# re-ovo/wgpu-path-tracing

Hardware: AMD Instinct MI355X
Metric: Msamples/s (rays x bounces / s) (higher is better)
Workload: dtype f32

## Files before the change

### wgpu-path-tracing_amd/csrc/dispatch.hip

```cpp
#include "ptmi_ctx.h"

#include <algorithm>
#include <cmath>
#include <cstring>
#include <utility>
#include <vector>

namespace {

constexpr size_t kMaxPendingEvents = 4096;
constexpr size_t kMaxDispatchesInFlight = 256;

const struct { double ptmi_stats::*ms; uint64_t ptmi_stats::*launches; } kEventStat[kEventKinds] = {
    {&ptmi_stats::gpu_ms, nullptr},
    {&ptmi_stats::extend_ms, &ptmi_stats::extend_launches},
    {&ptmi_stats::shade_ms, &ptmi_stats::shade_launches},
    {&ptmi_stats::shadow_ms, &ptmi_stats::shadow_launches},
    {&ptmi_stats::raygen_ms, nullptr},
    {&ptmi_stats::compact_ms, nullptr},
    {&ptmi_stats::accumulate_ms, nullptr},
};

hipEvent_t get_event(ptmi_ctx *c) {
    if (!c->event_pool.empty()) { hipEvent_t e = c->event_pool.back(); c->event_pool.pop_back(); return e; }
// ... 135 lines not shown
        float4 *const aov_rec = c->aov_mask ? ln.aov : nullptr;
        float4 *const mom = plane_as<float4>(c, kMoments);
        unsigned long long *const ct = c->d_counters;
        uint32_t *const qlen = &c->d_control[kCwQueue], *const slen = &c->d_control[kCwShadow];
        if (ap && !map && cam->frame_index == 0u) { pt_launch_adaptive_restart(ms, blocks, band, mom); c->ad_rounds = 0; }
        auto batch = [&](uint32_t frame0, uint32_t fb) -> int {
            const DevPixels px = ap ? DevPixels{band, 0u, c->ad.list, &c->d_control[kCwAdActive], mom, &ct[kCtAdTraced]}
                                    : DevPixels{band, frame0, nullptr, nullptr, nullptr, nullptr};
            { Timed t(c, kRaygen, t3, ms); pt_launch_raygen(ms, blocks, *cam, px, fb, bp, &qlen[0]); }
            int cur = 0;
            for (uint32_t b = 0; b < maxb; b++) {
                const bool tail = b > rb;
                const uint32_t *q = b == 0 || b == rb + 1 ? nullptr : ln.queue[cur];
                const DevPaths sp = tail ? tp : bp;
                const int par = side ? (int)(b & 1u) : 0;
                const ShadeParams shp{b, maxb, c->opt.do_mis, ct, side ? 1u : 0u, tail ? ln.pid : nullptr};
                { Timed t(c, kExtend, t2, ms); launch_extend(c, ms, cfg, sp, q, &qlen[b], ln.hits);
                  if (alpha) alpha_resolve_paths(c, ms, cfg, sp, q, &qlen[b], ln.hits, nullptr); }
                const bool last = b + 1 == maxb;
                if (side && b >= 2) HIP_TRY(c, hipStreamWaitEvent(ms, ln.ev_shadow[par], 0));
                { Timed t(c, kShade, t3, ms);
                  (c->opt.perf_mode ? pt_launch_shade_fast : pt_launch_shade)(
                      ms, shade_blocks, c->sc, sp, q, &qlen[b], ln.hits, ln.sh[par], ln.alive, ln.shadowm, shp,
                      b == 0 ? aov_rec : nullptr); }
                { Timed t(c, kCompact, t3, ms);
                  pt_launch_compact(ms, tiles, q, &qlen[b], ln.alive, nee ? ln.shadowm : nullptr,
                                    ln.word_off, ln.queue[cur ^ 1], &qlen[b + 1], ln.sq[par], &slen[par],
                                    ct, b, last ? 0 : 1);
                  if (b == rb && !last) pt_launch_repack(ms, blocks, &qlen[b + 1], ln.queue[cur ^ 1], bp, tp, ln.pid); }
                if (side) {
                    HIP_TRY(c, hipEventRecord(ln.ev_ready, ms));
                    HIP_TRY(c, hipStreamWaitEvent(ss, ln.ev_ready, 0));
                    { Timed t(c, kShadow, t3, ss); launch_shadow(c, ss, cfg_shadow, bp, ln.sh[par], ln.sq[par], &slen[par], nullptr); }
                    HIP_TRY(c, hipEventRecord(ln.ev_shadow[par], ss));
                } else if (nee) {
                    Timed t(c, kShadow, t3, ms);
                    if (alpha) alpha_shadow_stage(c, ms, cfg, bp, ln.sh[0], ln.sq[0], &slen[0], ln.hits, nullptr, nullptr);
                    else launch_shadow(c, ms, cfg_shadow, bp, ln.sh[0], ln.sq[0], &slen[0], nullptr);
                }
                cur ^= 1;
            }
// ... 222 lines not shown
```

### wgpu-path-tracing_amd/csrc/pipeline.hip

```cpp
#include "pt_device.h"
#include "pt_math.h"

namespace {

constexpr int BLOCK = 256;

PT_DEV v3 camera_dir(const ptmi_camera &cam, float px, float py) {
    float uvx = (px / (float)cam.width) * 2.0f - 1.0f;
    float uvy = (py / (float)cam.height) * 2.0f - 1.0f;
    float th = tan1(cam.fov * 0.5f);
    v3 fw = mk3(cam.forward[0], cam.forward[1], cam.forward[2]);
    v3 rt = mk3(cam.right[0], cam.right[1], cam.right[2]);
    v3 up = mk3(cam.up[0], cam.up[1], cam.up[2]);
    v3 a = scale3(scale3(scale3(rt, uvx), th), cam.aspect);
    v3 b = scale3(scale3(up, uvy), th);
    return normalize3(add3(add3(fw, a), b));
}

PT_DEV void camera_ray(const ptmi_camera &cam, uint32_t x, uint32_t y, uint32_t frame, v3 &org, v3 &dir,
                       uint32_t &rng) {
    rng = rng_seed(x, y, frame);
    float jx = rng_f(rng), jy = rng_f(rng);
    v3 rt = mk3(cam.right[0], cam.right[1], cam.right[2]);
    v3 up = mk3(cam.up[0], cam.up[1], cam.up[2]);
// ... 63 lines not shown
__global__ __launch_bounds__(BLOCK) void k_raygen_list(ptmi_camera cam, uint32_t n, const uint32_t *xs,
                                                       const uint32_t *ys, const uint32_t *frames, DevPaths P) {
    uint32_t p = blockIdx.x * BLOCK + threadIdx.x;
    if (p >= n) return;
    v3 o, d; uint32_t rng;
    camera_ray(cam, xs[p], ys[p], frames[p], o, d, rng);
    init_path(P, p, o, d, rng);
}

#ifndef PT_TILE_WORDS
#define PT_TILE_WORDS 1024
#endif
constexpr int TILE_WORDS = PT_TILE_WORDS;
constexpr int TILE_WAVES = TILE_WORDS / 64;

__global__ __launch_bounds__(TILE_WORDS) void k_tile_sums(const uint32_t *__restrict__ count_ptr,
                                                          const uint64_t *__restrict__ alive,
                                                          const uint64_t *__restrict__ shadow,
                                                          uint32_t *__restrict__ tile_sums,
                                                          uint32_t *__restrict__ shadow_tile_sums,
                                                          unsigned long long *__restrict__ stats, uint32_t bounce) {
    __shared__ uint32_t wsum[TILE_WAVES], wssum[TILE_WAVES];
    const uint32_t count = *count_ptr;
    const uint32_t nwords = (count + 63u) >> 6;
    if (blockIdx.x == 0 && threadIdx.x == 0) {
        atomicAdd(&stats[kCtSegments], (unsigned long long)count); atomicAdd(&stats[kCtByBounce + bounce], (unsigned long long)count);
    }
    if (blockIdx.x * TILE_WORDS >= nwords) return;
    const uint32_t w = blockIdx.x * TILE_WORDS + threadIdx.x;
    uint32_t c = 0, sc = 0;
    if (w < nwords) { c = (uint32_t)__popcll(alive[w]); if (shadow) sc = (uint32_t)__popcll(shadow[w]); }
    for (int off = 32; off > 0; off >>= 1) { c += __shfl_down(c, off); sc += __shfl_down(sc, off); }
    if ((threadIdx.x & 63u) == 0u) { wsum[threadIdx.x >> 6] = c; wssum[threadIdx.x >> 6] = sc; }
    __syncthreads();
    if (threadIdx.x == 0) {
        uint32_t t = 0, ts = 0;
        for (int i = 0; i < TILE_WAVES; i++) { t += wsum[i]; ts += wssum[i]; }
        tile_sums[blockIdx.x] = t;
        shadow_tile_sums[blockIdx.x] = ts;
        if (ts) { atomicAdd(&stats[kCtShadowRays], (unsigned long long)ts); atomicAdd(&stats[kCtShadowTraced], (unsigned long long)ts); }
    }
}

template <bool PACKED>
PT_DEV void scatter_tile(uint32_t tile, const uint32_t *__restrict__ count_ptr, const uint32_t *__restrict__ queue,
                         const uint64_t *__restrict__ alive, const uint32_t *__restrict__ tile_sums,
                         uint32_t *__restrict__ next_queue, uint32_t *__restrict__ next_count) {
    __shared__ uint32_t wtot[TILE_WAVES];
    __shared__ uint32_t tile_base;
    const uint32_t count = *count_ptr;
    const uint32_t nwords = (count + 63u) >> 6;
    const uint32_t ntiles = (nwords + TILE_WORDS - 1) / TILE_WORDS;
    if (tile >= ntiles) {
        if (ntiles == 0 && tile == 0 && threadIdx.x == 0) *next_count = 0;
        return;
    }
    const uint32_t lane = threadIdx.x & 63u, wave = threadIdx.x >> 6;
    uint32_t pre = 0;
    for (uint32_t t = threadIdx.x; t < tile; t += TILE_WORDS) pre += tile_sums[t];
    for (int off = 32; off > 0; off >>= 1) pre += __shfl_down(pre, off);
    if (lane == 0) wtot[wave] = pre;
    __syncthreads();
    if (threadIdx.x == 0) { uint32_t t = 0; for (int i = 0; i < TILE_WAVES; i++) t += wtot[i]; tile_base = t; }
    __syncthreads();
    const uint32_t base0 = tile_base;
    __syncthreads();
    const uint32_t w = tile * TILE_WORDS + threadIdx.x;
    const uint64_t m = w < nwords ? alive[w] : 0ull;
    const uint32_t c = (uint32_t)__popcll(m);
    uint32_t inc = c;
    for (int off = 1; off < 64; off <<= 1) { uint32_t v = __shfl_up(inc, off); if (lane >= (uint32_t)off) inc += v; }
    if (lane == 63u) wtot[wave] = inc;
    __syncthreads();
    uint32_t wbase = 0;
    for (uint32_t i = 0; i < wave; i++) wbase += wtot[i];
    const uint32_t my_off = base0 + wbase + inc - c;
    if (tile == ntiles - 1 && threadIdx.x == TILE_WORDS - 1) *next_count = my_off + c;
    const uint32_t mlo = (uint32_t)m, mhi = (uint32_t)(m >> 32);
    const uint32_t w0 = tile * TILE_WORDS + wave * 64u;
    for (uint32_t j = 0; j < 64u; j++) {
        const uint32_t jlo = __shfl(mlo, (int)j), jhi = __shfl(mhi, (int)j), jbase = __shfl(my_off, (int)j);
        const uint64_t jm = ((uint64_t)jhi << 32) | jlo;
        if (jm == 0ull) continue;
        if ((jm >> lane) & 1ull) {
            const uint32_t below = (uint32_t)__popcll(jm & ((1ull << lane) - 1ull));
            const uint32_t slot = (w0 + j) * 64u + lane;
            next_queue[jbase + below] = PACKED ? (w0 + j) * 64u + below : queue ? queue[slot] : slot;
        }
    }
}

__global__ __launch_bounds__(TILE_WORDS) void k_scatter(const uint32_t *__restrict__ count_ptr,
                                                        const uint32_t *__restrict__ queue,
                                                        const uint64_t *__restrict__ alive,
                                                        const uint32_t *__restrict__ tile_sums,
                                                        uint32_t *__restrict__ next_queue,
                                                        uint32_t *__restrict__ next_count) {
    scatter_tile<false>(blockIdx.x, count_ptr, queue, alive, tile_sums, next_queue, next_count);
}
__global__ __launch_bounds__(TILE_WORDS) void k_scatter_packed(const uint32_t *__restrict__ count_ptr,
                                                               const uint64_t *__restrict__ shadow,
                                                               const uint32_t *__restrict__ shadow_sums,
                                                               uint32_t *__restrict__ shadow_queue,
                                                               uint32_t *__restrict__ shadow_count) {
    scatter_tile<true>(blockIdx.x, count_ptr, nullptr, shadow, shadow_sums, shadow_queue, shadow_count);
}
__global__ __launch_bounds__(TILE_WORDS) void k_scatter2(uint32_t tiles, const uint32_t *__restrict__ count_ptr,
                                                         const uint32_t *__restrict__ queue,
                                                         const uint64_t *__restrict__ alive, const uint64_t *__restrict__ shadow,
                                                         const uint32_t *__restrict__ tile_sums, const uint32_t *__restrict__ shadow_sums,
                                                         uint32_t *__restrict__ next_queue, uint32_t *__restrict__ next_count,
                                                         uint32_t *__restrict__ shadow_queue, uint32_t *__restrict__ shadow_count) {
    if (blockIdx.x < tiles) scatter_tile<false>(blockIdx.x, count_ptr, queue, alive, tile_sums, next_queue, next_count);
    else scatter_tile<true>(blockIdx.x - tiles, count_ptr, nullptr, shadow, shadow_sums, shadow_queue, shadow_count);
}

__global__ __launch_bounds__(BLOCK) void k_repack(const uint32_t *__restrict__ count_ptr, const uint32_t *__restrict__ queue,
                                                  DevPaths from, DevPaths to, uint32_t *__restrict__ pid) {
    const uint32_t n = *count_ptr;
    for (uint32_t j = blockIdx.x * BLOCK + threadIdx.x; j < n; j += gridDim.x * BLOCK) {
        const uint32_t q = queue[j];
        const float4 o = ld_stream(&from.O[q]), d = ld_stream(&from.D[q]);
        const float2 c = ld_stream(&from.C[q]);
        st_stream(&to.O[j], o); st_stream(&to.D[j], d); st_stream(&to.C[j], c);
        if (from.W) to.W[j] = from.W[q];
        pid[j] = q;
    }
}

// ... 164 lines not shown
    const uint32_t nwords = (*count_ptr + 63u) >> 6;
    const uint32_t w = blockIdx.x * TILE_WORDS + threadIdx.x;
    uint32_t c = w < nwords ? (uint32_t)__popcll(ballot[w]) : 0u;
    for (int off = 32; off > 0; off >>= 1) c += __shfl_down(c, off);
    if ((threadIdx.x & 63u) == 0u) wsum[threadIdx.x >> 6] = c;
    __syncthreads();
    if (threadIdx.x == 0) {
        uint32_t t = 0;
        for (int i = 0; i < TILE_WAVES; i++) t += wsum[i];
        tile_sums[blockIdx.x] = t;
    }
}
__global__ __launch_bounds__(TILE_WORDS) void k_ad_scatter(const uint32_t *__restrict__ count_ptr, const uint64_t *__restrict__ ballot,
                                                           const uint32_t *__restrict__ tile_sums, uint32_t *__restrict__ list,
                                                           uint32_t *__restrict__ n_active) {
    scatter_tile<false>(blockIdx.x, count_ptr, nullptr, ballot, tile_sums, list, n_active);
}

__global__ __launch_bounds__(BLOCK) void k_ad_raygen(ptmi_camera cam, DevBand band, const uint32_t *__restrict__ list,
                                                     const uint32_t *__restrict__ n_active, uint32_t n_frames,
                                                     const float4 *__restrict__ mom, DevPaths P, uint32_t *__restrict__ count_out,
                                                     unsigned long long *__restrict__ traced) {
    if (blockIdx.x == 0 && threadIdx.x == 0) atomicAdd(traced, (unsigned long long)(*n_active * n_frames));
    raygen(cam, ListedPixels{band, list, n_active, mom}, n_frames, P, count_out);
}
__global__ __launch_bounds__(BLOCK) void k_ad_accumulate(DevBand band, const uint32_t *__restrict__ list, const uint32_t *__restrict__ n_active,
                                                         uint32_t n_frames, const float4 *__restrict__ mom, const float *__restrict__ L,
                                                         uint32_t l_stride, float4 *__restrict__ out) {
    fold_radiance(ListedPixels{band, list, n_active, mom}, n_frames, L, l_stride, out);
}
__global__ __launch_bounds__(BLOCK) void k_ad_accumulate_aov(DevBand band, const uint32_t *__restrict__ list, const uint32_t *__restrict__ n_active,
// ... 159 lines not shown
void pt_launch_raygen(hipStream_t s, int blocks, const ptmi_camera &cam, DevPixels px, uint32_t n_frames, DevPaths p,
                      uint32_t *count_out) {
    if (px.list)
        hipLaunchKernelGGL(k_ad_raygen, dim3(blocks), dim3(BLOCK), 0, s, cam, px.band, px.list, px.n_active, n_frames, px.mom, p, count_out,
                           px.traced);
    else hipLaunchKernelGGL(k_raygen, dim3(blocks), dim3(BLOCK), 0, s, cam, px.band, px.frame0, n_frames, p, count_out);
}
void pt_launch_center_rays(hipStream_t s, int blocks, const ptmi_camera &cam, DevBand band, DevPaths p, uint32_t *count_out) {
    hipLaunchKernelGGL(k_center_rays, dim3(blocks), dim3(BLOCK), 0, s, cam, band, p, count_out);
}
void pt_launch_raygen_list(hipStream_t s, const ptmi_camera &cam, uint32_t n, const uint32_t *xs,
                           const uint32_t *ys, const uint32_t *frames, DevPaths p) {
    hipLaunchKernelGGL(k_raygen_list, dim3((n + BLOCK - 1) / BLOCK), dim3(BLOCK), 0, s, cam, n, xs, ys, frames, p);
}
void pt_launch_compact(hipStream_t s, int tiles, const uint32_t *queue, const uint32_t *count,
                       const uint64_t *alive_mask, const uint64_t *shadow_mask, uint32_t *tile_sums,
                       uint32_t *next_queue, uint32_t *next_count, uint32_t *shadow_queue, uint32_t *shadow_count,
                       unsigned long long *stats, uint32_t bounce, int do_scatter) {
    uint32_t *shadow_sums = tile_sums + tiles;
    hipLaunchKernelGGL(k_tile_sums, dim3(tiles), dim3(TILE_WORDS), 0, s, count, alive_mask, shadow_mask, tile_sums,
                       shadow_sums, stats, bounce);
#ifndef PT_NO_SCATTER2
    if (do_scatter && shadow_mask) {
        hipLaunchKernelGGL(k_scatter2, dim3(2 * tiles), dim3(TILE_WORDS), 0, s, (uint32_t)tiles, count, queue, alive_mask, shadow_mask,
                           tile_sums, shadow_sums, next_queue, next_count, shadow_queue, shadow_count);
        return;
    }
#endif
    if (do_scatter)
        hipLaunchKernelGGL(k_scatter, dim3(tiles), dim3(TILE_WORDS), 0, s, count, queue, alive_mask, tile_sums,
                           next_queue, next_count);
    if (shadow_mask)
        hipLaunchKernelGGL(k_scatter_packed, dim3(tiles), dim3(TILE_WORDS), 0, s, count, shadow_mask, shadow_sums, shadow_queue,
                           shadow_count);
}
void pt_launch_repack(hipStream_t s, int blocks, const uint32_t *count, const uint32_t *queue, DevPaths from, DevPaths to,
                      uint32_t *pid) {
    hipLaunchKernelGGL(k_repack, dim3(blocks), dim3(BLOCK), 0, s, count, queue, from, to, pid);
}
void pt_launch_accumulate(hipStream_t s, int blocks, DevPixels px, uint32_t n_frames, const float *L, uint32_t l_stride, float4 *out) {
    if (px.list)
        hipLaunchKernelGGL(k_ad_accumulate, dim3(blocks), dim3(BLOCK), 0, s, px.band, px.list, px.n_active, n_frames, px.mom, L, l_stride, out);
    else hipLaunchKernelGGL(k_accumulate, dim3(blocks), dim3(BLOCK), 0, s, px.band, px.frame0, n_frames, L, l_stride, out);
}
void pt_launch_accumulate_aov(hipStream_t s, int blocks, DevPixels px, uint32_t n_frames, const float4 *rec,
                              const ptmi_triangle *tris, uint32_t n_tris, float4 *albedo, float4 *normal, uint2 *ids) {
    if (px.list)
        hipLaunchKernelGGL(k_ad_accumulate_aov, dim3(blocks), dim3(BLOCK), 0, s, px.band, px.list, px.n_active, n_frames, px.mom, rec, tris,
                           n_tris, albedo, normal, ids);
// ... 51 lines not shown
```

### wgpu-path-tracing_amd/csrc/pt_device.h

```cpp
#pragma once
#include <hip/hip_runtime.h>
#include <stdint.h>
#include <initializer_list>
#include "ptmi_layout.h"
#include "ptmi.h"

#define PT_HD __host__ __device__ inline

#define PT_REF_LEAF      0x80000000u
#define PT_REF_NONE      0xFFFFFFFFu
#define PT_LEAF_MAX_TRIS 32u
#define PT_LEAF_OFF_BITS 26u
#define PT_LEAF_OFF_MASK ((1u << PT_LEAF_OFF_BITS) - 1u)

struct DevEnv {
    const float4 *tab;
    const uint2 *alias;
    uint32_t w, h;
    uint32_t sampled;
    float intensity, rotation;
};

struct DevMedium {
    float sigma_t, g;
// ... 121 lines not shown
static_assert(kCtDispatchEnd - kCtByBounce == 64 && sizeof(ptmi_stats::segments_by_bounce) == 64 * sizeof(uint64_t),
              "a word per bounce up to max_bounces' limit, as ptmi_stats reports them");
static_assert(kCwShadow - kCwQueue == 64 + 1, "bounce b reads queue length b and writes b + 1, for b < 64");
static_assert(kCtAdTraced < kCtDispatchEnd && kCtAdSum >= kCtDispatchEnd && kCtRpCarried >= kCtDispatchEnd,
              "ptmi_reset_stats zeroes the dispatch statistics and the adaptive traced count, nothing else");
static_assert(kCtAlphaPathPasses > kCtSegments && kCtAlphaShadowExhausted == kCtAlphaPathPasses + 3 && kCtAlphaShadowExhausted < kCtDispatchEnd,
              "ptmi_reset_stats zeroes the four alpha counters, ptmi_alpha_status reads them with one copy");
static_assert(kCtAdMin == kCtAdSum + 1 && kCtAdMax == kCtAdSum + 2, "ptmi_adaptive_status presets and reads the three with one copy each");
static_assert(kCtRpDisoccluded == kCtRpCarried + 1 && kCtRpMissed == kCtRpCarried + 2 && kCtRpSamples == kCtRpCarried + 3,
              "ptmi_reproject zeroes the four with one memset, ptmi_reproject_status reads them with one copy");
static_assert(kCtRpMoved == kCtRpSamples + 1 && kCtRpMovedCarried == kCtRpMoved + 1,
              "the two motion words follow the four: the same memset zeroes all six, ptmi_motion_status reads the two with one copy");

struct ShadeParams {
    uint32_t bounce, max_bounces, do_mis;
    unsigned long long *stats;
    uint32_t emit_records;
    const uint32_t *pid;
};

enum { PT_VARIANT_GLOBAL = 1, PT_VARIANT_LDS = 2, PT_VARIANT_LDS_NODES = 3,
       PT_VARIANT_OWN_LDS = 4, PT_VARIANT_OWN_LDS_NODES = 5, PT_VARIANT_OWN_QLDS = 6, PT_VARIANT_OWN_QLDS_NODES = 7,
       PT_VARIANT_OWN_QGLOBAL = 8, PT_VARIANT_OWN_GLOBAL = 9,
       PT_VARIANT_OWN_LDS16_NODES = 10,
       PT_VARIANT_OWN_QLDS16_NODES = 11,
       PT_VARIANT_COUNT };

enum PtNodes {
    PT_NODES_EXACT,
    PT_NODES_QUANT,
    PT_NODES_EXACT16,
// ... 81 lines not shown
void pt_launch_hit_uv(hipStream_t s, uint32_t n, const DevScene &sc, DevPaths p, const float2 *hits, float2 *uv);
void pt_launch_shadow(hipStream_t s, int blocks, const TraverseConfig &cfg, const DevScene &sc, DevPaths p,
                      DevShadow sh, const uint32_t *shadow_queue, const uint32_t *count, uint8_t *occluded_out);
void pt_launch_shadow_own(hipStream_t s, int blocks, const TraverseConfig &cfg, const DevScene &sc, DevPaths p,
                          DevShadow sh, const uint32_t *shadow_queue, const uint32_t *count, uint8_t *occluded_out);
void pt_launch_shade(hipStream_t s, int blocks, const DevScene &sc, DevPaths p, const uint32_t *queue,
                     const uint32_t *count, const float2 *hits, DevShadow sh, uint64_t *alive_mask,
                     uint64_t *shadow_mask, ShadeParams sp, float4 *aov = nullptr);
void pt_launch_shade_fast(hipStream_t s, int blocks, const DevScene &sc, DevPaths p, const uint32_t *queue,
                          const uint32_t *count, const float2 *hits, DevShadow sh, uint64_t *alive_mask,
                          uint64_t *shadow_mask, ShadeParams sp, float4 *aov = nullptr);
uint32_t pt_compact_tile_slots(void);
void pt_launch_repack(hipStream_t s, int blocks, const uint32_t *count, const uint32_t *queue, DevPaths from, DevPaths to,
                      uint32_t *pid);
void pt_launch_compact(hipStream_t s, int tiles, const uint32_t *queue, const uint32_t *count,
                       const uint64_t *alive_mask, const uint64_t *shadow_mask, uint32_t *tile_sums,
                       uint32_t *next_queue, uint32_t *next_count, uint32_t *shadow_queue, uint32_t *shadow_count,
                       unsigned long long *stats, uint32_t bounce, int do_scatter);
void pt_launch_accumulate(hipStream_t s, int blocks, DevPixels px, uint32_t n_frames, const float *L, uint32_t l_stride, float4 *out);
void pt_launch_accumulate_aov(hipStream_t s, int blocks, DevPixels px, uint32_t n_frames, const float4 *rec,
                              const ptmi_triangle *tris, uint32_t n_tris, float4 *albedo, float4 *normal, uint2 *ids);
void pt_launch_accumulate_moments(hipStream_t s, int blocks, DevPixels px, uint32_t n_frames, const float *L, uint32_t l_stride,
                                  float4 *mom);
struct DevAdaptive {
    uint64_t *ballot;
    uint32_t *list;
    uint32_t *tile_sums;
    uint32_t *control;
    unsigned long long *counters;
};
uint32_t pt_adaptive_tiles(uint32_t npix);
// ... 55 lines not shown
```

### wgpu-path-tracing_amd/csrc/ptmi_api.hip

```cpp
#include "ptmi_ctx.h"

#include <algorithm>
#include <cmath>
#include <cstdarg>
#include <cstdio>
#include <cstring>

namespace {

void vfail(std::string &err, const char *fmt, va_list ap) {
    char buf[512];
    vsnprintf(buf, sizeof buf, fmt, ap);
    err = buf;
}

constexpr size_t kLaneBytes[kLaneBufs] = {
    16, 16, 8, 16,
    8,
    16 + 16 + sizeof(rgb_sc), 4, 16 + 16 + sizeof(rgb_sc), 4,
    16, 16, 8, 4,
    4, 4,
    1,
    32,
    4, 4,
    16, 16, 4, 4, 8,
};
constexpr bool lane_buf_wanted(int k, bool aov, bool env_w, bool alpha) {
    return k == kAovRec ? aov : k == kPathW || k == kTailW ? env_w : k >= kAlphaO && k <= kAlphaHits ? alpha : true;
}
constexpr size_t lane_bytes_per_path(bool aov, bool env_w, bool alpha) {
    size_t n = 1;
    for (int k = 0; k < kLaneBufs; k++) if (lane_buf_wanted(k, aov, env_w, alpha)) n += kLaneBytes[k];
    return n;
}
static_assert(lane_bytes_per_path(false, false, false) == 214 && lane_bytes_per_path(true, false, false) == 246 &&
              lane_bytes_per_path(false, true, false) == 222 && lane_bytes_per_path(false, false, true) == 262,
              "the automatic frames_per_batch moves with these");

}

PT_HOST {
void lane_views(Lane &ln) {
    auto at = [&](int k, auto *&p) { view(p, ln.buf[k]); };
    at(kPathO, ln.paths.O); at(kPathD, ln.paths.D); at(kPathC, ln.paths.C); at(kPathL, ln.paths.L);
    at(kHits, ln.hits);
    for (int k = 0; k < 2; k++) {
        DevShadow &sh = ln.sh[k];
        at(k ? kShadow1 : kShadow0, sh.SO); at(k ? kShadowIdx1 : kShadowIdx0, ln.sq[k]); at(k ? kQueue1 : kQueue0, ln.queue[k]);
        sh.SD = sh.SO ? sh.SO + ln.cap : nullptr; sh.SC = sh.SO ? reinterpret_cast<rgb_sc *>(sh.SO + 2 * ln.cap) : nullptr;
        sh.cap = (uint32_t)ln.cap;
    }
    at(kTailO, ln.tail.O); at(kTailD, ln.tail.D); at(kTailC, ln.tail.C); at(kPid, ln.pid);
    at(kOcc, ln.d_occ); at(kAovRec, ln.aov);
    at(kPathW, ln.paths.W); at(kTailW, ln.tail.W);
    at(kAlphaO, ln.alpha.RO); at(kAlphaD, ln.alpha.RD); at(kAlphaList0, ln.alpha.list[0]); at(kAlphaList1, ln.alpha.list[1]);
    at(kAlphaHits, ln.alpha.hits);
}
}

namespace {

void free_batch(Lane &ln) {
    for (void *&p : ln.buf) dfree(p);
    dfree(ln.alive); dfree(ln.shadowm); dfree(ln.word_off);
    ln.cap = 0;
    lane_views(ln);
}

uint32_t stats_depth(const ptmi_ctx *c) { return c->img.leaves_used == 2u ? c->img.ref_depth : std::max(c->img.depth, c->img.ref_depth); }

constexpr uint32_t kAovAll = PTMI_AOV_ALBEDO | PTMI_AOV_NORMAL | PTMI_AOV_ID;

template <size_t K> size_t per_pixel(size_t px) { return px * K; }
size_t ballot_bytes(size_t px) { return (px / 64 + 1) * 8; }
size_t tile_sum_bytes(size_t px) { return (size_t)pt_adaptive_tiles((uint32_t)px) * 4; }
const struct { const char *name; size_t (*bytes)(size_t px); bool zeroed; PlaneGroup group; } kFrame[kFramePlanes] = {
    {"output", per_pixel<PTMI_OUTPUT_STRIDE>, true, kWithFrame},
    {"albedo", per_pixel<16>, true, kWithFrame}, {"normal", per_pixel<16>, true, kWithFrame}, {"id", per_pixel<8>, true, kWithFrame},
    {"moments", per_pixel<16>, true, kWithFrame},
// ... 65 lines not shown
hipError_t sync_all(ptmi_ctx *c) {
    hipError_t e = c->stream ? hipStreamSynchronize(c->stream) : hipSuccess;
    if (e == hipSuccess && c->lane.side) e = hipStreamSynchronize(c->lane.side);
    if (e == hipSuccess && c->stream) e = hipStreamSynchronize(c->stream);
    return e;
}

size_t bytes_per_path(bool aov, bool env_w, bool alpha) { return lane_bytes_per_path(aov, env_w, alpha); }

int ensure_capacity(ptmi_ctx *c, Lane &ln, size_t n) {
    const bool aov = c->aov_mask != 0, env_w = c->sc.env.sampled != 0, alpha = alpha_active(c);
    if (n <= ln.cap && (!aov || ln.aov) && (!env_w || ln.paths.W) && (!alpha || ln.alpha.RO)) return PTMI_OK;
    HIP_TRY(c, sync_all(c));
    free_batch(ln);
    const size_t cap = (n + 1023) & ~(size_t)1023;
    const size_t words = cap / 64 + 1;
    const size_t tiles = cap / pt_compact_tile_slots() + 2;
    c->alloc_oom = false;
    hipError_t e = hipSuccess;
    size_t bytes = 0;
    for (int k = 0; k < kLaneBufs && e == hipSuccess; k++)
        if (lane_buf_wanted(k, aov, env_w, alpha)) e = hipMalloc(&ln.buf[k], bytes = cap * kLaneBytes[k]);
    if (e == hipSuccess) e = hipMalloc(&ln.alive, bytes = words * 8);
    if (e == hipSuccess) e = hipMalloc(&ln.shadowm, bytes = words * 8);
    if (e == hipSuccess) e = hipMalloc(&ln.word_off, bytes = 2 * tiles * 4);
    if (e != hipSuccess) {
        c->alloc_oom = e == hipErrorOutOfMemory;
        free_batch(ln);
        (void)hipGetLastError();
        return fail(c, PTMI_E_HIP, "hipMalloc of %zu bytes for a batch of %zu paths failed: %s", bytes, cap, hipGetErrorString(e));
    }
    ln.mask_words = words;
    ln.cap = cap;
    lane_views(ln);
    return PTMI_OK;
}

size_t plane_bytes(FramePlane k, size_t px) { return kFrame[k].bytes(px); }
uint32_t group_set(PlaneGroup g) {
    uint32_t set = 0;
    for (int k = 0; k < kFramePlanes; k++) if (kFrame[k].group == g) set |= 1u << k;
    return set;
}

int make_planes(ptmi_ctx *c, uint32_t set, size_t px, void **into) {
    void *n[kFramePlanes] = {};
    for (int k = 0; k < kFramePlanes && px; k++) {
// ... 420 lines not shown
```

### wgpu-path-tracing_amd/csrc/ptmi_ctx.h

```cpp
#pragma once
#include "ptmi.h"
#include "pt_device.h"

#include <chrono>
#include <cstddef>
#include <cstdint>
#include <deque>
#include <string>
#include <vector>

struct ptmi_ctx;
struct PtPrepared;
PtPrepared *pt_prepare_scene(ptmi_ctx *c, const ptmi_triangle *tris, uint32_t nt, const ptmi_material *mats, uint32_t nm,
                             const ptmi_bvh_node *nodes, uint32_t nn, const ptmi_light *lights, uint32_t nl, int *rc_out);
int pt_install_scene(ptmi_ctx *c, PtPrepared *p);
void pt_free_prepared(PtPrepared *p);
int pt_atlas_bytes(uint32_t width, uint32_t height, int format, size_t *bytes, char *why, size_t why_len);
int pt_check_medium(const ptmi_medium *m, std::string &err);
int pt_check_medium_depth(const ptmi_medium *m, std::string &err);
int pt_check_medium_density(const float *rho, uint32_t nx, uint32_t ny, uint32_t nz, const ptmi_medium_grid *params,
                            struct ptmi_medium_grid_status *st, std::string &err);
const ptmi_medium *pt_ctx_medium(const ptmi_ctx *c);
bool pt_ctx_has_medium_grid(const ptmi_ctx *c);
int pt_check_alpha_cutoff(const float *cutoff, uint32_t n_materials, const ptmi_alpha_params *params, std::string &err);
// ... 44 lines not shown
    kBlitF32, kBlitU8,
    kMotion,
    kFramePlanes
};

enum LaneBuf {
    kPathO, kPathD, kPathC, kPathL,
    kHits,
    kShadow0, kShadowIdx0, kShadow1, kShadowIdx1,
    kTailO, kTailD, kTailC, kPid,
    kQueue0, kQueue1,
    kOcc,
    kAovRec,
    kPathW, kTailW,
    kAlphaO, kAlphaD, kAlphaList0, kAlphaList1, kAlphaHits,
    kLaneBufs
};

enum EventKind { kDispatch, kExtend, kShade, kShadow, kRaygen, kCompact, kAccumulate, kEventKinds };
struct EventPair { hipEvent_t a, b; EventKind kind; };

}
using namespace pt_host;

struct Lane {
    size_t cap = 0;
    void *buf[kLaneBufs] = {};
    DevPaths paths{};
    float2 *hits = nullptr;
    DevShadow sh[2]{};
    uint32_t *queue[2] = {nullptr, nullptr}, *sq[2] = {nullptr, nullptr};
    DevPaths tail{};
    uint32_t *pid = nullptr;
    uint64_t *alive = nullptr, *shadowm = nullptr;
    size_t mask_words = 0;
    uint32_t *word_off = nullptr;
    uint32_t *d_spill = nullptr;
    uint32_t *d_spill_side = nullptr;
    uint8_t *d_occ = nullptr;
    hipStream_t side = nullptr;
    hipEvent_t ev_ready = nullptr, ev_shadow[2] = {nullptr, nullptr};
    float4 *aov = nullptr;
    DevAlpha alpha{};
};

struct ptmi_ctx {
    int device = 0, n_cu = 256;
    hipStream_t own_stream = nullptr, stream = nullptr;
    Lane lane;
    mutable std::string err;
// ... 123 lines not shown
```

### wgpu-path-tracing_amd/csrc/shade.hip

```cpp
#include "pt_device.h"
#include "pt_math.h"
#include "pt_hit.h"
#include "pt_texel.h"
#include "pt_env.h"
#include "pt_medium.h"

namespace {

struct HitInfo {
    v3 position; float t;
    v3 normal;
    v3 albedo;
    float roughness, metallic, transmission, ior;
    v3 emission; float emissive_strength;
    bool is_front;
};

typedef float f4v __attribute__((ext_vector_type(4)));
typedef const __attribute__((address_space(3))) f4v *lds_f4p;
template <class R, int Q> PT_DEV R lds_record(lds_f4p p) {
    static_assert(sizeof(R) == Q * 16, "a record of Q quads");
    R r;
    __builtin_memcpy(&r, p, sizeof r);
    return r;
// ... 307 lines not shown
                                                  uint64_t *__restrict__ alive_mask,
                                                  uint64_t *__restrict__ shadow_mask, ShadeParams sp,
                                                  float4 *__restrict__ aov) {
    extern __shared__ float4 smem[];
    const uint32_t count = *count_ptr;
    const uint32_t lane = threadIdx.x & 63u;
    const uint32_t mats_q = (STAGE & PT_STAGE_MATS) ? (uint32_t)pt_tab_mats_q(sc.n_mats) : 0u;
    const uint32_t lights_q = (STAGE & PT_STAGE_LIGHTS) ? (uint32_t)pt_tab_lights_q(sc.n_lights) : 0u;
    if (STAGE) {
        const float4 *src = sc.shade_tab + ((STAGE & PT_STAGE_MATS) ? 0u : pt_tab_mats_q(sc.n_mats));
        for (uint32_t k = threadIdx.x; k < mats_q + lights_q; k += SBLOCK) smem[k] = src[k];
        __syncthreads();
    }
    const lds_f4p lds_lights = (lds_f4p)smem + mats_q;
    const ShadeTabs<STAGE> tabs{(lds_f4p)smem, lds_lights, lds_lights + 3u * sc.n_lights};
    uint32_t n_skipped = 0, n_emitted = 0;
    for (uint32_t base = blockIdx.x * SBLOCK; base < count; base += gridDim.x * SBLOCK) {
        const uint32_t i = base + threadIdx.x;
        bool alive = false, shadow = false, skipped = false, emitted = false;
        float4 rec_o = make_float4(0.0f, 0.0f, 0.0f, -2.0f), rec_d = make_float4(0.0f, 0.0f, 0.0f, 0.0f);
        rgb_sc rec_c{0.0f, 0.0f, 0.0f};
        if (i < count) {
            const uint32_t q = queue ? queue[i] : i;
            const float2 h2 = ld_stream(&hits[i]);
            bool scattered = false;
            uint32_t med_rng = 0u;
            float4 med_o4 = make_float4(0.0f, 0.0f, 0.0f, 0.0f), med_d4 = med_o4;
            if (MED) {
                med_o4 = ld_stream(&P.O[q]); med_d4 = ld_stream(&P.D[q]);
                const float4 o4 = med_o4, d4 = med_d4;
                const v3 ro = xyz(o4), rd = xyz(d4);
// ... 134 lines not shown
                    const v3 e = mk3(tx * 0.0f, c2.x * 0.0f, c2.y * 0.0f);
                    if (terminal_add(P, sp.emit_records, p, e, rec_d, rec_c)) { shadow = true; emitted = true; }
                }
            }
        }
        const uint64_t am = __ballot(alive), sm = __ballot(shadow), zm = __ballot(skipped), em = __ballot(emitted);
        if (shadow) {
            const uint32_t r = (i & ~63u) + (uint32_t)__popcll(sm & ((1ull << lane) - 1ull));
            st_stream(&S.SO[r], rec_o);
            st_stream(&S.SD[r], rec_d);
            S.SC[r] = rec_c;
        }
        if (lane == 0u && i < count) {
            alive_mask[i >> 6] = am;
            shadow_mask[i >> 6] = sm;
            n_skipped += (uint32_t)__popcll(zm);
            n_emitted += (uint32_t)__popcll(em);
        }
    }
    if (n_skipped) atomicAdd(&sp.stats[kCtShadowRays], (unsigned long long)n_skipped);
    if (n_emitted) atomicAdd(&sp.stats[kCtEmitRecords], (unsigned long long)n_emitted);
}

}

#ifdef PT_SHADE_FAST
#define PT_LAUNCH_SHADE pt_launch_shade_fast
#else
#define PT_LAUNCH_SHADE pt_launch_shade
#endif
namespace {
template <bool AOV, int STAGE, bool ENV, int MED>
void launch_shade(hipStream_t s, int blocks, const DevScene &sc, DevPaths p, const uint32_t *queue, const uint32_t *count,
                  const float2 *hits, DevShadow sh, uint64_t *alive_mask, uint64_t *shadow_mask, ShadeParams sp, float4 *aov) {
    const size_t lds = (((STAGE & PT_STAGE_MATS) ? pt_tab_mats_q(sc.n_mats) : 0) + ((STAGE & PT_STAGE_LIGHTS) ? pt_tab_lights_q(sc.n_lights) : 0)) * 16;
    hipLaunchKernelGGL((k_shade<AOV, STAGE, ENV, MED>), dim3(blocks), dim3(SBLOCK), lds, s, sc, p, queue, count, hits, sh, alive_mask,
// ... 22 lines not shown
```

Baseline: 12010.

## Replace per-block shade stat atomics with per-word counts reduced in compaction

The shade kernel no longer issues per-block 64-bit atomicAdds for skipped shadow rays and emit records. It writes a packed per-wave-word count, which the tile-sum and scatter kernels reduce and add once from the last tile. This removes global atomic contention at the end of shade, and also turns the per-tile shadow atomics into a single add. The cost is an extra count buffer read in compaction, more LDS and reduction work, and mask and tile-sum buffers are now allocated through the lane buffer table.

```diff
diff --git a/wgpu-path-tracing_amd/csrc/dispatch.hip b/wgpu-path-tracing_amd/csrc/dispatch.hip
--- a/wgpu-path-tracing_amd/csrc/dispatch.hip
+++ b/wgpu-path-tracing_amd/csrc/dispatch.hip
@@ -173,7 +173,7 @@
                 const uint32_t *q = b == 0 || b == rb + 1 ? nullptr : ln.queue[cur];
                 const DevPaths sp = tail ? tp : bp;
                 const int par = side ? (int)(b & 1u) : 0;
-                const ShadeParams shp{b, maxb, c->opt.do_mis, ct, side ? 1u : 0u, tail ? ln.pid : nullptr};
+                const ShadeParams shp{b, maxb, c->opt.do_mis, ln.counts, side ? 1u : 0u, tail ? ln.pid : nullptr};
                 { Timed t(c, kExtend, t2, ms); launch_extend(c, ms, cfg, sp, q, &qlen[b], ln.hits);
                   if (alpha) alpha_resolve_paths(c, ms, cfg, sp, q, &qlen[b], ln.hits, nullptr); }
                 const bool last = b + 1 == maxb;
@@ -183,7 +183,7 @@
                       ms, shade_blocks, c->sc, sp, q, &qlen[b], ln.hits, ln.sh[par], ln.alive, ln.shadowm, shp,
                       b == 0 ? aov_rec : nullptr); }
                 { Timed t(c, kCompact, t3, ms);
-                  pt_launch_compact(ms, tiles, q, &qlen[b], ln.alive, nee ? ln.shadowm : nullptr,
+                  pt_launch_compact(ms, tiles, q, &qlen[b], ln.alive, nee ? ln.shadowm : nullptr, ln.counts,
                                     ln.word_off, ln.queue[cur ^ 1], &qlen[b + 1], ln.sq[par], &slen[par],
                                     ct, b, last ? 0 : 1);
                   if (b == rb && !last) pt_launch_repack(ms, blocks, &qlen[b + 1], ln.queue[cur ^ 1], bp, tp, ln.pid); }
diff --git a/wgpu-path-tracing_amd/csrc/pipeline.hip b/wgpu-path-tracing_amd/csrc/pipeline.hip
--- a/wgpu-path-tracing_amd/csrc/pipeline.hip
+++ b/wgpu-path-tracing_amd/csrc/pipeline.hip
@@ -101,13 +101,18 @@
 constexpr int TILE_WORDS = PT_TILE_WORDS;
 constexpr int TILE_WAVES = TILE_WORDS / 64;
 
+struct TileStats {
+    const uint32_t *skipped, *emitted;
+    unsigned long long *stats;
+};
+
 __global__ __launch_bounds__(TILE_WORDS) void k_tile_sums(const uint32_t *__restrict__ count_ptr,
                                                           const uint64_t *__restrict__ alive,
                                                           const uint64_t *__restrict__ shadow,
+                                                          const uint32_t *__restrict__ counts,
                                                           uint32_t *__restrict__ tile_sums,
-                                                          uint32_t *__restrict__ shadow_tile_sums,
-                                                          unsigned long long *__restrict__ stats, uint32_t bounce) {
-    __shared__ uint32_t wsum[TILE_WAVES], wssum[TILE_WAVES];
+                                                          unsigned long long *__restrict__ stats, uint32_t bounce, int add_here) {
+    __shared__ uint32_t wsum[TILE_WAVES], wssum[TILE_WAVES], wcsum[TILE_WAVES];
     const uint32_t count = *count_ptr;
     const uint32_t nwords = (count + 63u) >> 6;
     if (blockIdx.x == 0 && threadIdx.x == 0) {
@@ -115,26 +120,30 @@
     }
     if (blockIdx.x * TILE_WORDS >= nwords) return;
     const uint32_t w = blockIdx.x * TILE_WORDS + threadIdx.x;
-    uint32_t c = 0, sc = 0;
-    if (w < nwords) { c = (uint32_t)__popcll(alive[w]); if (shadow) sc = (uint32_t)__popcll(shadow[w]); }
-    for (int off = 32; off > 0; off >>= 1) { c += __shfl_down(c, off); sc += __shfl_down(sc, off); }
-    if ((threadIdx.x & 63u) == 0u) { wsum[threadIdx.x >> 6] = c; wssum[threadIdx.x >> 6] = sc; }
+    uint32_t c = 0, sc = 0, zc = 0;
+    if (w < nwords) { c = (uint32_t)__popcll(alive[w]); if (shadow) sc = (uint32_t)__popcll(shadow[w]); zc = counts[w]; }
+    for (int off = 32; off > 0; off >>= 1) { c += __shfl_down(c, off); sc += __shfl_down(sc, off); zc += __shfl_down(zc, off); }
+    if ((threadIdx.x & 63u) == 0u) { wsum[threadIdx.x >> 6] = c; wssum[threadIdx.x >> 6] = sc; wcsum[threadIdx.x >> 6] = zc; }
     __syncthreads();
     if (threadIdx.x == 0) {
-        uint32_t t = 0, ts = 0;
-        for (int i = 0; i < TILE_WAVES; i++) { t += wsum[i]; ts += wssum[i]; }
+        uint32_t t = 0, ts = 0, tz = 0, te = 0;
+        for (int i = 0; i < TILE_WAVES; i++) { t += wsum[i]; ts += wssum[i]; tz += wcsum[i] & 0xFFFFu; te += wcsum[i] >> 16; }
+        const uint32_t tiles = gridDim.x;
         tile_sums[blockIdx.x] = t;
-        shadow_tile_sums[blockIdx.x] = ts;
-        if (ts) { atomicAdd(&stats[kCtShadowRays], (unsigned long long)ts); atomicAdd(&stats[kCtShadowTraced], (unsigned long long)ts); }
+        tile_sums[tiles + blockIdx.x] = ts;
+        tile_sums[2u * tiles + blockIdx.x] = tz;
+        tile_sums[3u * tiles + blockIdx.x] = te;
+        if (add_here && tz) atomicAdd(&stats[kCtShadowRays], (unsigned long long)tz);
+        if (add_here && te) atomicAdd(&stats[kCtEmitRecords], (unsigned long long)te);
     }
 }
 
 template <bool PACKED>
 PT_DEV void scatter_tile(uint32_t tile, const uint32_t *__restrict__ count_ptr, const uint32_t *__restrict__ queue,
                          const uint64_t *__restrict__ alive, const uint32_t *__restrict__ tile_sums,
-                         uint32_t *__restrict__ next_queue, uint32_t *__restrict__ next_count) {
-    __shared__ uint32_t wtot[TILE_WAVES];
-    __shared__ uint32_t tile_base;
+                         uint32_t *__restrict__ next_queue, uint32_t *__restrict__ next_count, TileStats st) {
+    __shared__ uint32_t wtot[TILE_WAVES], wskip[TILE_WAVES], wemit[TILE_WAVES];
+    __shared__ uint32_t tile_base, all_skipped, all_emitted;
     const uint32_t count = *count_ptr;
     const uint32_t nwords = (count + 63u) >> 6;
     const uint32_t ntiles = (nwords + TILE_WORDS - 1) / TILE_WORDS;
@@ -143,12 +152,19 @@
         return;
     }
     const uint32_t lane = threadIdx.x & 63u, wave = threadIdx.x >> 6;
-    uint32_t pre = 0;
+    const bool adds = st.stats && tile == ntiles - 1;
+    uint32_t pre = 0, nz = 0, ne = 0;
     for (uint32_t t = threadIdx.x; t < tile; t += TILE_WORDS) pre += tile_sums[t];
+    if (adds) for (uint32_t t = threadIdx.x; t < ntiles; t += TILE_WORDS) { nz += st.skipped[t]; ne += st.emitted[t]; }
     for (int off = 32; off > 0; off >>= 1) pre += __shfl_down(pre, off);
-    if (lane == 0) wtot[wave] = pre;
+    if (adds) for (int off = 32; off > 0; off >>= 1) { nz += __shfl_down(nz, off); ne += __shfl_down(ne, off); }
+    if (lane == 0) { wtot[wave] = pre; wskip[wave] = nz; wemit[wave] = ne; }
     __syncthreads();
-    if (threadIdx.x == 0) { uint32_t t = 0; for (int i = 0; i < TILE_WAVES; i++) t += wtot[i]; tile_base = t; }
+    if (threadIdx.x == 0) {
+        uint32_t t = 0, z = 0, e = 0;
+        for (int i = 0; i < TILE_WAVES; i++) { t += wtot[i]; z += wskip[i]; e += wemit[i]; }
+        tile_base = t; all_skipped = z; all_emitted = e;
+    }
     __syncthreads();
     const uint32_t base0 = tile_base;
     __syncthreads();
@@ -162,7 +178,15 @@
     uint32_t wbase = 0;
     for (uint32_t i = 0; i < wave; i++) wbase += wtot[i];
     const uint32_t my_off = base0 + wbase + inc - c;
-    if (tile == ntiles - 1 && threadIdx.x == TILE_WORDS - 1) *next_count = my_off + c;
+    if (tile == ntiles - 1 && threadIdx.x == TILE_WORDS - 1) {
+        const uint32_t listed = my_off + c;
+        *next_count = listed;
+        if (adds) {
+            atomicAdd(&st.stats[kCtShadowRays], (unsigned long long)(PACKED ? listed : 0u) + all_skipped);
+            if (PACKED) atomicAdd(&st.stats[kCtShadowTraced], (unsigned long long)listed);
+            atomicAdd(&st.stats[kCtEmitRecords], (unsigned long long)all_emitted);
+        }
+    }
     const uint32_t mlo = (uint32_t)m, mhi = (uint32_t)(m >> 32);
     const uint32_t w0 = tile * TILE_WORDS + wave * 64u;
     for (uint32_t j = 0; j < 64u; j++) {
@@ -182,24 +206,25 @@
                                                         const uint64_t *__restrict__ alive,
                                                         const uint32_t *__restrict__ tile_sums,
                                                         uint32_t *__restrict__ next_queue,
-                                                        uint32_t *__restrict__ next_count) {
-    scatter_tile<false>(blockIdx.x, count_ptr, queue, alive, tile_sums, next_queue, next_count);
+                                                        uint32_t *__restrict__ next_count, TileStats st) {
+    scatter_tile<false>(blockIdx.x, count_ptr, queue, alive, tile_sums, next_queue, next_count, st);
 }
 __global__ __launch_bounds__(TILE_WORDS) void k_scatter_packed(const uint32_t *__restrict__ count_ptr,
                                                                const uint64_t *__restrict__ shadow,
                                                                const uint32_t *__restrict__ shadow_sums,
                                                                uint32_t *__restrict__ shadow_queue,
-                                                               uint32_t *__restrict__ shadow_count) {
-    scatter_tile<true>(blockIdx.x, count_ptr, nullptr, shadow, shadow_sums, shadow_queue, shadow_count);
+                                                               uint32_t *__restrict__ shadow_count, TileStats st) {
+    scatter_tile<true>(blockIdx.x, count_ptr, nullptr, shadow, shadow_sums, shadow_queue, shadow_count, st);
 }
 __global__ __launch_bounds__(TILE_WORDS) void k_scatter2(uint32_t tiles, const uint32_t *__restrict__ count_ptr,
                                                          const uint32_t *__restrict__ queue,
                                                          const uint64_t *__restrict__ alive, const uint64_t *__restrict__ shadow,
                                                          const uint32_t *__restrict__ tile_sums, const uint32_t *__restrict__ shadow_sums,
                                                          uint32_t *__restrict__ next_queue, uint32_t *__restrict__ next_count,
-                                                         uint32_t *__restrict__ shadow_queue, uint32_t *__restrict__ shadow_count) {
-    if (blockIdx.x < tiles) scatter_tile<false>(blockIdx.x, count_ptr, queue, alive, tile_sums, next_queue, next_count);
-    else scatter_tile<true>(blockIdx.x - tiles, count_ptr, nullptr, shadow, shadow_sums, shadow_queue, shadow_count);
+                                                         uint32_t *__restrict__ shadow_queue, uint32_t *__restrict__ shadow_count,
+                                                         TileStats st) {
+    if (blockIdx.x < tiles) scatter_tile<false>(blockIdx.x, count_ptr, queue, alive, tile_sums, next_queue, next_count, TileStats{});
+    else scatter_tile<true>(blockIdx.x - tiles, count_ptr, nullptr, shadow, shadow_sums, shadow_queue, shadow_count, st);
 }
 
 __global__ __launch_bounds__(BLOCK) void k_repack(const uint32_t *__restrict__ count_ptr, const uint32_t *__restrict__ queue,
@@ -394,7 +419,7 @@
 __global__ __launch_bounds__(TILE_WORDS) void k_ad_scatter(const uint32_t *__restrict__ count_ptr, const uint64_t *__restrict__ ballot,
                                                            const uint32_t *__restrict__ tile_sums, uint32_t *__restrict__ list,
                                                            uint32_t *__restrict__ n_active) {
-    scatter_tile<false>(blockIdx.x, count_ptr, nullptr, ballot, tile_sums, list, n_active);
+    scatter_tile<false>(blockIdx.x, count_ptr, nullptr, ballot, tile_sums, list, n_active, TileStats{});
 }
 
 __global__ __launch_bounds__(BLOCK) void k_ad_raygen(ptmi_camera cam, DevBand band, const uint32_t *__restrict__ list,
@@ -584,25 +609,26 @@
     hipLaunchKernelGGL(k_raygen_list, dim3((n + BLOCK - 1) / BLOCK), dim3(BLOCK), 0, s, cam, n, xs, ys, frames, p);
 }
 void pt_launch_compact(hipStream_t s, int tiles, const uint32_t *queue, const uint32_t *count,
-                       const uint64_t *alive_mask, const uint64_t *shadow_mask, uint32_t *tile_sums,
+                       const uint64_t *alive_mask, const uint64_t *shadow_mask, const uint32_t *counts, uint32_t *tile_sums,
                        uint32_t *next_queue, uint32_t *next_count, uint32_t *shadow_queue, uint32_t *shadow_count,
                        unsigned long long *stats, uint32_t bounce, int do_scatter) {
     uint32_t *shadow_sums = tile_sums + tiles;
-    hipLaunchKernelGGL(k_tile_sums, dim3(tiles), dim3(TILE_WORDS), 0, s, count, alive_mask, shadow_mask, tile_sums,
-                       shadow_sums, stats, bounce);
+    const TileStats st{tile_sums + 2 * tiles, tile_sums + 3 * tiles, stats}, none{};
+    hipLaunchKernelGGL(k_tile_sums, dim3(tiles), dim3(TILE_WORDS), 0, s, count, alive_mask, shadow_mask, counts, tile_sums,
+                       stats, bounce, !do_scatter && !shadow_mask);
 #ifndef PT_NO_SCATTER2
     if (do_scatter && shadow_mask) {
         hipLaunchKernelGGL(k_scatter2, dim3(2 * tiles), dim3(TILE_WORDS), 0, s, (uint32_t)tiles, count, queue, alive_mask, shadow_mask,
-                           tile_sums, shadow_sums, next_queue, next_count, shadow_queue, shadow_count);
+                           tile_sums, shadow_sums, next_queue, next_count, shadow_queue, shadow_count, st);
         return;
     }
 #endif
     if (do_scatter)
         hipLaunchKernelGGL(k_scatter, dim3(tiles), dim3(TILE_WORDS), 0, s, count, queue, alive_mask, tile_sums,
-                           next_queue, next_count);
+                           next_queue, next_count, shadow_mask ? none : st);
     if (shadow_mask)
         hipLaunchKernelGGL(k_scatter_packed, dim3(tiles), dim3(TILE_WORDS), 0, s, count, shadow_mask, shadow_sums, shadow_queue,
-                           shadow_count);
+                           shadow_count, st);
 }
 void pt_launch_repack(hipStream_t s, int blocks, const uint32_t *count, const uint32_t *queue, DevPaths from, DevPaths to,
                       uint32_t *pid) {
diff --git a/wgpu-path-tracing_amd/csrc/pt_device.h b/wgpu-path-tracing_amd/csrc/pt_device.h
--- a/wgpu-path-tracing_amd/csrc/pt_device.h
+++ b/wgpu-path-tracing_amd/csrc/pt_device.h
@@ -159,7 +159,7 @@
 
 struct ShadeParams {
     uint32_t bounce, max_bounces, do_mis;
-    unsigned long long *stats;
+    uint32_t *counts;
     uint32_t emit_records;
     const uint32_t *pid;
 };
@@ -271,7 +271,7 @@
 void pt_launch_repack(hipStream_t s, int blocks, const uint32_t *count, const uint32_t *queue, DevPaths from, DevPaths to,
                       uint32_t *pid);
 void pt_launch_compact(hipStream_t s, int tiles, const uint32_t *queue, const uint32_t *count,
-                       const uint64_t *alive_mask, const uint64_t *shadow_mask, uint32_t *tile_sums,
+                       const uint64_t *alive_mask, const uint64_t *shadow_mask, const uint32_t *counts, uint32_t *tile_sums,
                        uint32_t *next_queue, uint32_t *next_count, uint32_t *shadow_queue, uint32_t *shadow_count,
                        unsigned long long *stats, uint32_t bounce, int do_scatter);
 void pt_launch_accumulate(hipStream_t s, int blocks, DevPixels px, uint32_t n_frames, const float *L, uint32_t l_stride, float4 *out);
diff --git a/wgpu-path-tracing_amd/csrc/ptmi_api.hip b/wgpu-path-tracing_amd/csrc/ptmi_api.hip
--- a/wgpu-path-tracing_amd/csrc/ptmi_api.hip
+++ b/wgpu-path-tracing_amd/csrc/ptmi_api.hip
@@ -24,13 +24,18 @@
     32,
     4, 4,
     16, 16, 4, 4, 8,
+    8, 8, 4,
+    4 * 4,
 };
+size_t lane_elements(int k, size_t cap) {
+    return k < kLanePerPath ? cap : k == kTileSums ? cap / pt_compact_tile_slots() + 2 : cap / 64 + 1;
+}
 constexpr bool lane_buf_wanted(int k, bool aov, bool env_w, bool alpha) {
     return k == kAovRec ? aov : k == kPathW || k == kTailW ? env_w : k >= kAlphaO && k <= kAlphaHits ? alpha : true;
 }
 constexpr size_t lane_bytes_per_path(bool aov, bool env_w, bool alpha) {
     size_t n = 1;
-    for (int k = 0; k < kLaneBufs; k++) if (lane_buf_wanted(k, aov, env_w, alpha)) n += kLaneBytes[k];
+    for (int k = 0; k < kLanePerPath; k++) if (lane_buf_wanted(k, aov, env_w, alpha)) n += kLaneBytes[k];
     return n;
 }
 static_assert(lane_bytes_per_path(false, false, false) == 214 && lane_bytes_per_path(true, false, false) == 246 &&
@@ -55,6 +60,7 @@
     at(kPathW, ln.paths.W); at(kTailW, ln.tail.W);
     at(kAlphaO, ln.alpha.RO); at(kAlphaD, ln.alpha.RD); at(kAlphaList0, ln.alpha.list[0]); at(kAlphaList1, ln.alpha.list[1]);
     at(kAlphaHits, ln.alpha.hits);
+    at(kAliveMask, ln.alive); at(kShadowMask, ln.shadowm); at(kShadeCounts, ln.counts); at(kTileSums, ln.word_off);
 }
 }
 
@@ -62,7 +68,6 @@
 
 void free_batch(Lane &ln) {
     for (void *&p : ln.buf) dfree(p);
-    dfree(ln.alive); dfree(ln.shadowm); dfree(ln.word_off);
     ln.cap = 0;
     lane_views(ln);
 }
@@ -158,23 +163,17 @@
     HIP_TRY(c, sync_all(c));
     free_batch(ln);
     const size_t cap = (n + 1023) & ~(size_t)1023;
-    const size_t words = cap / 64 + 1;
-    const size_t tiles = cap / pt_compact_tile_slots() + 2;
     c->alloc_oom = false;
     hipError_t e = hipSuccess;
     size_t bytes = 0;
     for (int k = 0; k < kLaneBufs && e == hipSuccess; k++)
-        if (lane_buf_wanted(k, aov, env_w, alpha)) e = hipMalloc(&ln.buf[k], bytes = cap * kLaneBytes[k]);
-    if (e == hipSuccess) e = hipMalloc(&ln.alive, bytes = words * 8);
-    if (e == hipSuccess) e = hipMalloc(&ln.shadowm, bytes = words * 8);
-    if (e == hipSuccess) e = hipMalloc(&ln.word_off, bytes = 2 * tiles * 4);
+        if (lane_buf_wanted(k, aov, env_w, alpha)) e = hipMalloc(&ln.buf[k], bytes = lane_elements(k, cap) * kLaneBytes[k]);
     if (e != hipSuccess) {
         c->alloc_oom = e == hipErrorOutOfMemory;
         free_batch(ln);
         (void)hipGetLastError();
         return fail(c, PTMI_E_HIP, "hipMalloc of %zu bytes for a batch of %zu paths failed: %s", bytes, cap, hipGetErrorString(e));
     }
-    ln.mask_words = words;
     ln.cap = cap;
     lane_views(ln);
     return PTMI_OK;
diff --git a/wgpu-path-tracing_amd/csrc/ptmi_ctx.h b/wgpu-path-tracing_amd/csrc/ptmi_ctx.h
--- a/wgpu-path-tracing_amd/csrc/ptmi_ctx.h
+++ b/wgpu-path-tracing_amd/csrc/ptmi_ctx.h
@@ -82,7 +82,11 @@
     kAovRec,
     kPathW, kTailW,
     kAlphaO, kAlphaD, kAlphaList0, kAlphaList1, kAlphaHits,
-    kLaneBufs
+    kAliveMask, kShadowMask,
+    kShadeCounts,
+    kTileSums,
+    kLaneBufs,
+    kLanePerPath = kAliveMask
 };
 
 enum EventKind { kDispatch, kExtend, kShade, kShadow, kRaygen, kCompact, kAccumulate, kEventKinds };
@@ -101,7 +105,7 @@
     DevPaths tail{};
     uint32_t *pid = nullptr;
     uint64_t *alive = nullptr, *shadowm = nullptr;
-    size_t mask_words = 0;
+    uint32_t *counts = nullptr;
     uint32_t *word_off = nullptr;
     uint32_t *d_spill = nullptr;
     uint32_t *d_spill_side = nullptr;
diff --git a/wgpu-path-tracing_amd/csrc/shade.hip b/wgpu-path-tracing_amd/csrc/shade.hip
--- a/wgpu-path-tracing_amd/csrc/shade.hip
+++ b/wgpu-path-tracing_amd/csrc/shade.hip
@@ -345,7 +345,7 @@
     }
     const lds_f4p lds_lights = (lds_f4p)smem + mats_q;
     const ShadeTabs<STAGE> tabs{(lds_f4p)smem, lds_lights, lds_lights + 3u * sc.n_lights};
-    uint32_t n_skipped = 0, n_emitted = 0;
+    uint32_t *__restrict__ const count_words = sp.counts;
     for (uint32_t base = blockIdx.x * SBLOCK; base < count; base += gridDim.x * SBLOCK) {
         const uint32_t i = base + threadIdx.x;
         bool alive = false, shadow = false, skipped = false, emitted = false;
@@ -510,12 +510,9 @@
         if (lane == 0u && i < count) {
             alive_mask[i >> 6] = am;
             shadow_mask[i >> 6] = sm;
-            n_skipped += (uint32_t)__popcll(zm);
-            n_emitted += (uint32_t)__popcll(em);
+            count_words[i >> 6] = (uint32_t)__popcll(zm) | (uint32_t)__popcll(em) << 16;
         }
     }
-    if (n_skipped) atomicAdd(&sp.stats[kCtShadowRays], (unsigned long long)n_skipped);
-    if (n_emitted) atomicAdd(&sp.stats[kCtEmitRecords], (unsigned long long)n_emitted);
 }
 
 }
```

Measured after the change: 12340, median of 6. 2.8% higher.
